# bdwsq1996/Effi-MVS-plus

Measured on NVIDIA B200. Metric: depth_maps_per_sec_1600x1184_5view, higher is better.
Workload: dtype hi+lo bf16 MMA x3, f32 accumulate (3-D regularization, fp32-grade) / f32 (warp, lookup, regression)

## Files before the change

### effi-mvs-plus_b200/capi.py

```python
from __future__ import annotations

import ctypes as C
import os

_HERE = os.path.dirname(os.path.abspath(__file__))
LIB_PATH = os.environ.get("EFFIMVS_LIB") or os.path.join(_HERE, "libeffimvs.so")

OK, EINVAL, EUNSUPPORTED, ECUDA, EWORKSPACE = 0, -1, -2, -3, -4
HYP_TENSOR, HYP_PLANES, HYP_LOCAL = 0, 1, 2
RANGE_SCALAR, RANGE_PIXEL = 0, 1
FEA_NCHW, FEA_NHWC = 0, 1
PREC_F32, PREC_BF16, PREC_BF16X3 = 0, 1, 2
WS_PREPARE, WS_RUN = 1, 2
CONV2D_BIAS, CONV2D_BIAS_RELU, CONV2D_ADD_RELU, CONV2D_GRU_GATES, CONV2D_GRU_UPDATE = 0, 1, 2, 3, 4
MAX_SRC_VIEWS = 16


class EffiMVSError(RuntimeError):
    def __init__(self, code, msg):
        super().__init__("libeffimvs error {}: {}".format(code, msg))
        self.code = code


if not os.path.exists(LIB_PATH):
# ... 34 lines not shown
    "effimvs_inv_init_f32": (_i, [_p, _p, _p, _i, _i, _p, _p, _p]),
    "effimvs_delta_head_f32": (_i, [_p, _p, _p, _p, _p, _p, _i, _i, _i, _i, _p, _p, _p]),
    "effimvs_convex_upsample_f32": (_i, [_p, _p, _f, _p, _p, _p, _i, _i, _i, _i, _p, _p, _p]),
    "effimvs_convex_upsample_conv_f32": (_i, [_p, _i, _p, _p, _f, _p, _p, _p, _i, _i, _i, _i, _p, _p, _p]),
    "effimvs_encoder_head_f32": (_i, [_p, _p, _p, _p, _p, _p, _i, _i, _i, _i, _i, _p, _p]),
    "effimvs_encoder_head_hostw_f32": (_i, [_p, _p, _p, _i, _i, _i, _i, _i, _p, _p]),
    "effimvs_encoder_head_pack_host": (_i, [_p, _p, _p, _p, _i, _i, _p]),
    "effimvs_encoder_head_table_floats": (_i, [_i]),
    "effimvs_encoder_tail_f32": (_i, [_p, _p, _p, C.c_longlong, _i, _i, _p, _p]),
    "effimvs_encoder_tail_ctx_f32": (_i, [_p, _p, _p, _i, _i, _i, _p, _p, C.c_longlong, _i, _i, _p, _p]),
    "effimvs_conv2d_tf32_supported": (_i, [_i, _i]),
    "effimvs_conv2d_tf32_packed_bytes": (_sz, [_i, _i]),
    "effimvs_conv2d_tf32_pack": (_i, [_p, _i, _i, _p, _p]),
    "effimvs_conv2d_tf32": (_i, [_p, C.c_longlong, _i, _p, C.c_longlong, _i, _p, _p, _i, _i, _i, _i, _i,
                                 _p, C.c_longlong, _p, C.c_longlong, _p, C.c_longlong, _p]),
    "effimvs_gru_init_f32": (_i, [_p, C.c_longlong, _i, _i, _p, _p]),
    "effimvs_gru_init_ctx_f32": (_i, [_p, C.c_longlong, _i, _i, _p, _p, _p, _p, _p]),
    "effimvs_dtu_filter_f32": (_i, [_p, _p, _p, _p, C.POINTER(C.c_double), C.POINTER(C.c_float), _i, _i, _i, _f, _f, _i, _i, _i,
                                    _p, _p, _p, _p, _p, _p, _p]),
    "effimvs_images_u8_to_f32": (_i, [_p, C.c_longlong, _p, _p]),
    "effimvs_fusion_invert_cameras_f32": (_i, [_p, _p, _i, _i, _p, _p]),
    "effimvs_fusion_reproject_f32": (_i, [_p, _p, _p, _p, _p, _i, _i, _i, _i, _p, _p]),
    "effimvs_fusion_filter_f32": (_i, [_p, _p, _p, _p, _p, _p, _i, _i, _i, _i, _i, _i, _f, _f, _i, _f, _i, _p, _p, _p, _p, _p]),
}

for _name, (_res, _args) in SIGNATURES.items():
    _fn = getattr(lib, _name)
    _fn.restype = _res
    _fn.argtypes = _args

# ... 14 lines not shown
```

### effi-mvs-plus_b200/csrc/common.cuh

```cuda
#pragma once
#include <cuda_runtime.h>
#include <stdint.h>
#include <stdio.h>

#include <utility>

#include "../../include/effimvs.h"

namespace effimvs {

void set_error(const char* fmt, ...);

inline int check_launch(const char* what) {
    cudaError_t e = cudaGetLastError();
    if (e != cudaSuccess) {
        set_error("%s: %s", what, cudaGetErrorString(e));
        return EFFIMVS_ECUDA;
    }
    return EFFIMVS_OK;
}

#define EFFI_REQUIRE(cond, code, ...)      \
    do {                                   \
        if (!(cond)) {                     \
// ... 30 lines not shown
template <class... KArgs, class... Args>
inline void launch_kernel(void (*kernel)(KArgs...), dim3 grid, dim3 block, size_t smem, cudaStream_t stream, Args&&... args) {
    cudaLaunchConfig_t cfg = {};
    cfg.gridDim = grid;
    cfg.blockDim = block;
    cfg.dynamicSmemBytes = smem;
    cfg.stream = stream;
    cudaLaunchAttribute attr[1];
    attr[0].id = cudaLaunchAttributeProgrammaticStreamSerialization;
    attr[0].val.programmaticStreamSerializationAllowed = 1;
    cfg.attrs = attr;
    cfg.numAttrs = pdl_enabled() ? 1 : 0;
    cudaLaunchKernelEx(&cfg, kernel, std::forward<Args>(args)...);
}

struct SrcPtrs {
    const float* p[EFFIMVS_MAX_SRC_VIEWS];
};

}
```

### effi-mvs-plus_b200/csrc/conv2d_tc.cu

```cuda
#include <cuda_fp16.h>

#include <algorithm>
#include <cstdlib>

#include "common.cuh"

namespace effimvs {
namespace {

constexpr int C2_TM = 128;
constexpr int C2_ROWPX = 136;
constexpr int C2_CG_BYTES = C2_ROWPX * 16;
constexpr int C2_STAGES = 4;
constexpr int C2_RING = 16;
constexpr int C2_PROD_WARPS = 8;
constexpr int C2_PROD_GROUPS = 2;
constexpr int C2_GROUP_WARPS = C2_PROD_WARPS / C2_PROD_GROUPS;
constexpr int C2_MMA_WARP = 4, C2_PROD_WARP0 = 5;
constexpr int C2_THREADS = (C2_PROD_WARP0 + C2_PROD_WARPS) * 32;
constexpr int C2_EPI_STRIDE = 144;
constexpr int C2_EPI_BYTES = 4 * 32 * C2_EPI_STRIDE;
constexpr int C2_MAX_COUT = 128;

struct C2Params {
// ... 2 lines not shown
    int cin, cout, coutp;
    int B, H, W;
    int kc, n_phases;
    int strips, R, chunks, n_units;
    int mode;
    const float* bias;
    float* out; long long out_ps;
    const float* aux0; long long aux0_ps;
    float* aux1; long long aux1_ps;
    int tmem_cols, w_bytes, stage_bytes, n_stages;
    int gw;
    int ring;
    long long* tl;
    int debug;
};

__device__ __forceinline__ uint32_t smem_u32(const void* p) { return (uint32_t)__cvta_generic_to_shared(p); }
__device__ __forceinline__ void mbar_init(uint64_t* bar, uint32_t count) {
    asm volatile("mbarrier.init.shared::cta.b64 [%0], %1;" ::"r"(smem_u32(bar)), "r"(count));
}
__device__ __forceinline__ void mbar_expect_tx(uint64_t* bar, uint32_t bytes) {
    asm volatile("mbarrier.arrive.expect_tx.shared::cta.b64 _, [%0], %1;" ::"r"(smem_u32(bar)), "r"(bytes) : "memory");
}
__device__ __forceinline__ void mbar_arrive(uint64_t* bar) {
    asm volatile("mbarrier.arrive.shared::cta.b64 _, [%0];" ::"r"(smem_u32(bar)) : "memory");
}
__device__ __forceinline__ uint32_t mbar_try(uint64_t* bar, uint32_t parity) {
    uint32_t done;
    asm volatile(
        "{\n\t.reg .pred p;\n\t"
// ... 200 lines not shown
}

struct Unit { int b, y0, y1, x0; };
__device__ __forceinline__ Unit unit_of(const C2Params& P, int u) {
    Unit t;
    const int per_img = P.strips * P.chunks;
    t.b = u / per_img;
    const int r = u - t.b * per_img;
    const int chunk = r / P.strips, strip = r - chunk * P.strips;
    t.y0 = chunk * P.R;
    t.y1 = min(t.y0 + P.R, P.H);
    t.x0 = strip * C2_TM;
    return t;
}

template <int MODE, int GROUPS>
__global__ void __launch_bounds__(C2_THREADS, 2)
conv2d_tc_kernel(const __grid_constant__ C2Params P, const uint8_t* __restrict__ wpk) {
#ifdef EFFIMVS_CONV2D_PROFILING
    const int dbg = dbg;
#else
    constexpr int dbg = 0;
#endif
    constexpr int KC = GROUPS * 8;
    extern __shared__ __align__(128) uint8_t smem[];
    __shared__ __align__(8) uint64_t bar_afull[C2_STAGES], bar_aempty[C2_STAGES], bar_tfull[C2_RING], bar_tempty[C2_RING], bar_w;
    __shared__ uint32_t tmem_base_s;
    __shared__ __align__(16) float sbias[C2_MAX_COUT];
    const int tid = threadIdx.x, warp = __shfl_sync(0xffffffffu, tid >> 5, 0), lane = tid & 31;
    uint8_t* wsm = smem;
    uint8_t* astage = smem + P.w_bytes;

    if (warp == C2_MMA_WARP) {
// ... 4 lines not shown
        for (int s = 0; s < C2_STAGES; ++s) { mbar_init(&bar_afull[s], P.gw); mbar_init(&bar_aempty[s], 1); }
        for (int a = 0; a < C2_RING; ++a) { mbar_init(&bar_tfull[a], 1); mbar_init(&bar_tempty[a], 4); }
        mbar_init(&bar_w, 1);
        asm volatile("fence.mbarrier_init.release.cluster;" ::: "memory");
    }
    tc_fence_before();
    __syncthreads();
    tc_fence_after();
    if (tid == C2_PROD_WARP0 * 32) {
        mbar_expect_tx(&bar_w, (uint32_t)P.w_bytes);
        bulk_g2s(wsm, wpk, (uint32_t)P.w_bytes, &bar_w);
    }
    pdl_trigger();
    pdl_wait();
    if (tid < C2_MAX_COUT) sbias[tid] = (P.bias && tid < P.cout) ? __ldg(P.bias + tid) : 0.0f;
    __syncthreads();
    const uint32_t tmem = tmem_base_s;
    const int H = P.H, W = P.W;

    if (warp >= C2_PROD_WARP0) {
        const int pw = warp - C2_PROD_WARP0, grp = pw / P.gw, pwg = pw - grp * P.gw;
        const int S = P.n_stages;
        constexpr int groups = GROUPS;
        const int pxl = groups >= 4 ? (lane & 7) : (lane & 15), cgl0 = groups >= 4 ? (lane >> 3) : (lane >> 4);
        const int px_per_item = groups >= 4 ? 8 : 16, px_items = (C2_ROWPX + px_per_item - 1) / px_per_item;
        const int n_items = px_items * (groups >= 4 ? groups >> 2 : 1);
        const int ps0i = (int)P.ps0, ps1i = (int)P.ps1;
        uint32_t fill = 0;
        for (int u = blockIdx.x; u < P.n_units; u += gridDim.x) {
            const Unit t = unit_of(P, u);
            const int i_lo = max(t.y0 - 1, 0), i_hi = min(t.y1, H - 1);
            for (int i = i_lo; i <= i_hi; ++i) {
                const long long rowpix = ((long long)t.b * H + i) * W;
                for (int p = 0; p < P.n_phases; ++p, ++fill) {
                    if ((int)(fill % C2_PROD_GROUPS) != grp) continue;
// ... 212 lines not shown
        dst[i] = __float2half_rn(fminf(fmaxf(v, -65504.0f), 65504.0f));
    }
}

int pow2_cols(int n) { int c = 32; while (c < n) c <<= 1; return c; }
int phase_channels(int cin) { return (cin == 16 || cin == 32 || cin == 64) ? cin : (cin % 32 == 0 ? 32 : 16); }

}
}

using namespace effimvs;

static long long* g_conv2d_timeline = nullptr;
extern "C" void effimvs_conv2d_debug_timeline(void* buf) { g_conv2d_timeline = (long long*)buf; }

extern "C" size_t effimvs_conv2d_tf32_packed_bytes(int cin, int cout) {
    if (cin <= 0 || cout <= 0) return 0;
    const int coutp = (cout + 15) / 16 * 16;
    return (size_t)18 * cin * coutp;
}

extern "C" int effimvs_conv2d_tf32_supported(int cin, int cout) {
    if (cin < 16 || cin % 16 != 0 || cout < 4 || cout % 4 != 0 || cout > C2_MAX_COUT) return 0;
    const int coutp = (cout + 15) / 16 * 16;
    const int kc = phase_channels(cin);
    const size_t smem = (size_t)18 * cin * coutp + (size_t)3 * (kc / 8) * C2_CG_BYTES + C2_EPI_BYTES;
    if (smem > 224 * 1024) return 0;
    if (4 * coutp > 512) return 0;
    return 1;
}

extern "C" int effimvs_conv2d_tf32_pack(const float* w, int cin, int cout, void* packed, void* stream) {
    EFFI_REQUIRE(w && packed, EFFIMVS_EINVAL, "conv2d_tf32_pack: null pointer");
    EFFI_REQUIRE(effimvs_conv2d_tf32_supported(cin, cout), EFFIMVS_EUNSUPPORTED, "conv2d_tf32_pack: cin=%d cout=%d not supported", cin, cout);
    const int coutp = (cout + 15) / 16 * 16;
    const int total = 9 * cin * coutp;
    conv2d_pack_kernel<<<std::min(ceil_div(total, 256), 1024), 256, 0, (cudaStream_t)stream>>>(w, cin, cout, coutp, (__half*)packed);
    return check_launch("conv2d_pack_kernel");
}

extern "C" int effimvs_conv2d_tf32(const float* in0, long long in0_ps, int c0, const float* in1, long long in1_ps, int c1,
                                   const void* packed, const float* bias, int cout, int B, int H, int W, int mode,
                                   float* out, long long out_ps, const float* aux0, long long aux0_ps, float* aux1,
                                   long long aux1_ps, void* stream) {
    EFFI_REQUIRE(in0 && packed && out, EFFIMVS_EINVAL, "conv2d_tf32: null pointer");
    EFFI_REQUIRE(B > 0 && H >= 2 && W >= 1, EFFIMVS_EINVAL, "conv2d_tf32: bad shape %dx%dx%d", B, H, W);
    EFFI_REQUIRE(c0 > 0 && c0 % 8 == 0 && c1 >= 0 && c1 % 8 == 0 && (c1 == 0 || in1), EFFIMVS_EINVAL, "conv2d_tf32: bad channel segments %d + %d", c0, c1);
    const int cin = c0 + c1;
    EFFI_REQUIRE(effimvs_conv2d_tf32_supported(cin, cout), EFFIMVS_EUNSUPPORTED, "conv2d_tf32: cin=%d cout=%d not supported", cin, cout);
    EFFI_REQUIRE(mode >= EFFIMVS_CONV2D_BIAS && mode <= EFFIMVS_CONV2D_GRU_UPDATE, EFFIMVS_EINVAL, "conv2d_tf32: bad mode %d", mode);
    EFFI_REQUIRE(in0_ps >= c0 && in0_ps % 8 == 0 && (c1 == 0 || (in1_ps >= c1 && in1_ps % 8 == 0)) && out_ps % 4 == 0,
                 EFFIMVS_EINVAL, "conv2d_tf32: input pixel strides must be multiples of 8 floats, the output's of 4");
    EFFI_REQUIRE((((uintptr_t)in0 | (uintptr_t)in1) & 31) == 0 && (((uintptr_t)out | (uintptr_t)aux0 | (uintptr_t)aux1 | (uintptr_t)packed) & 15) == 0,
                 EFFIMVS_EINVAL, "conv2d_tf32: input maps must be 32-byte aligned, the other pointers 16-byte aligned");
    EFFI_REQUIRE((long long)W * in0_ps < (1ll << 31) && (long long)W * in1_ps < (1ll << 31), EFFIMVS_EUNSUPPORTED, "conv2d_tf32: a row of a map must be below 2^31 floats");
    if (mode == EFFIMVS_CONV2D_ADD_RELU) EFFI_REQUIRE(aux0 && aux0_ps % 4 == 0, EFFIMVS_EINVAL, "conv2d_tf32: ADD_RELU needs the addend map");
    if (mode == EFFIMVS_CONV2D_GRU_GATES)
        EFFI_REQUIRE(aux0 && aux1 && bias && cout % 32 == 0 && aux0_ps % 4 == 0 && aux1_ps % 4 == 0, EFFIMVS_EINVAL,
                     "conv2d_tf32: GRU_GATES needs h_prev, the z buffer, the bias and cout = 2h with h a multiple of 16");
    if (mode == EFFIMVS_CONV2D_GRU_UPDATE) EFFI_REQUIRE(aux0 && bias && aux0_ps % 4 == 0, EFFIMVS_EINVAL, "conv2d_tf32: GRU_UPDATE needs z and the bias");

    C2Params P;
    P.in0 = in0; P.ps0 = in0_ps; P.c0 = c0;
    P.in1 = in1 ? in1 : in0; P.ps1 = in1 ? in1_ps : in0_ps; P.c1 = c1;
    P.cin = cin; P.cout = cout; P.coutp = (cout + 15) / 16 * 16;
    P.B = B; P.H = H; P.W = W;
    P.kc = phase_channels(cin);
    P.n_phases = cin / P.kc;
    P.mode = mode;
    P.tl = g_conv2d_timeline;
    P.debug = getenv("EFFIMVS_CONV2D_DEBUG") ? atoi(getenv("EFFIMVS_CONV2D_DEBUG")) : 0;
    P.bias = bias;
    P.out = out; P.out_ps = out_ps;
    P.aux0 = aux0; P.aux0_ps = aux0_ps;
    P.aux1 = aux1; P.aux1_ps = aux1_ps;
    P.w_bytes = 18 * cin * P.coutp;
    P.stage_bytes = (P.kc / 8) * C2_CG_BYTES;
    const size_t fixed = (size_t)P.w_bytes + C2_EPI_BYTES;
    const size_t smem3 = fixed + 3 * (size_t)P.stage_bytes;
    int per_sm = smem3 + 1024 <= 75 * 1024 && 4 * P.coutp <= 128 ? 3 : (smem3 + 1024 <= 113 * 1024 && 4 * P.coutp <= 256 ? 2 : 1);
    if (const char* e = getenv("EFFIMVS_CONV2D_CTAS")) per_sm = std::max(1, std::min(per_sm, atoi(e)));
    P.gw = per_sm == 3 ? 2 : 4;
    const int tmem_budget = per_sm == 3 ? 128 : (per_sm == 2 ? 256 : 512);
    P.ring = 4;
    while (P.ring < C2_RING && 2 * P.ring * P.coutp <= tmem_budget) P.ring *= 2;
    if (const char* e = getenv("EFFIMVS_CONV2D_RING")) { int r = atoi(e); if ((r == 4 || r == 8 || r == 16) && r * P.coutp <= tmem_budget) P.ring = r; }
    P.tmem_cols = pow2_cols(P.ring * P.coutp);
    const size_t smem_budget = per_sm == 3 ? 75 * 1024 : (per_sm == 2 ? 113 * 1024 : 225 * 1024);
    P.n_stages = (smem3 + P.stage_bytes + 1024 <= smem_budget) ? 4 : 3;
    if (const char* e = getenv("EFFIMVS_CONV2D_STAGES")) { int n = atoi(e); if (n == 3 || (n == 4 && smem3 + P.stage_bytes + 1024 <= smem_budget)) P.n_stages = n; }
    const size_t smem = fixed + (size_t)P.n_stages * P.stage_bytes;
    const int G = kNumSMs * per_sm;
    P.strips = ceil_div(W, C2_TM);
    int chunks = std::max(1, (G + B * P.strips / 2) / (B * P.strips));
    if (const char* e = getenv("EFFIMVS_CONV2D_ROWS")) chunks = ceil_div(H, std::max(1, atoi(e)));
    int min_rows = 4;
    if (const char* e = getenv("EFFIMVS_CONV2D_MINROWS")) min_rows = std::max(1, atoi(e));
    P.R = std::max(std::min(min_rows, H), ceil_div(H, chunks));
    P.chunks = ceil_div(H, P.R);
    P.n_units = B * P.strips * P.chunks;

    typedef void (*KernelFn)(C2Params, const uint8_t*);
#define C2_ROW(M) {conv2d_tc_kernel<M, 2>, conv2d_tc_kernel<M, 4>, conv2d_tc_kernel<M, 8>}
    static const KernelFn table[5][3] = {C2_ROW(EFFIMVS_CONV2D_BIAS), C2_ROW(EFFIMVS_CONV2D_BIAS_RELU), C2_ROW(EFFIMVS_CONV2D_ADD_RELU),
                                         C2_ROW(EFFIMVS_CONV2D_GRU_GATES), C2_ROW(EFFIMVS_CONV2D_GRU_UPDATE)};
#undef C2_ROW
    const int gi = P.kc == 16 ? 0 : (P.kc == 32 ? 1 : 2);
    const KernelFn fn = table[mode][gi];
    static bool attr_set[64][5][3] = {};
    int dev = 0;
    cudaGetDevice(&dev);
    if (dev < 0 || dev >= 64 || !attr_set[dev][mode][gi]) {
        cudaError_t e = cudaFuncSetAttribute(fn, cudaFuncAttributeMaxDynamicSharedMemorySize, 226 * 1024);
        EFFI_REQUIRE(e == cudaSuccess, EFFIMVS_ECUDA, "conv2d_tf32: cudaFuncSetAttribute: %s", cudaGetErrorString(e));
        if (dev >= 0 && dev < 64) attr_set[dev][mode][gi] = true;
    }
    launch_kernel(fn, dim3(std::min(G, P.n_units)), dim3((C2_PROD_WARP0 + C2_PROD_GROUPS * P.gw) * 32), smem, (cudaStream_t)stream, P,
                  (const uint8_t*)packed);
    return check_launch("conv2d_tc_kernel");
}
```

### effi-mvs-plus_b200/csrc/update_glue.cu

```cuda
#include <stdlib.h>

#include "common.cuh"

namespace effimvs {
namespace {

__device__ __forceinline__ float sigmoid_t(float x) { return __fdiv_rn(1.0f, __fadd_rn(1.0f, expf(-x))); }

__device__ __forceinline__ float to_depth(float inv, float lo, float hi) {
    const float s = fmaxf(__fadd_rn(lo, __fmul_rn(__fsub_rn(hi, lo), inv)), 1e-4f);
    return __fdiv_rn(1.0f, s);
}

__global__ void __launch_bounds__(256)
gru_reset_kernel(const float4* __restrict__ zr_pre, const float* __restrict__ bias_r, const float4* __restrict__ hx, long long n_pix, int h,
                 int cx, float4* __restrict__ rhx) {
    pdl_enter();
    const int ct4 = (h + cx) >> 2, h4 = h >> 2;
    const long long total = n_pix * ct4;
    for (long long i = (long long)blockIdx.x * blockDim.x + threadIdx.x; i < total; i += (long long)gridDim.x * blockDim.x) {
        const long long p = i / ct4;
        const int c4 = (int)(i - p * ct4);
        float4 v = __ldg(hx + i);
        if (c4 < h4) {
// ... 412 lines not shown
                        acc[p][4 * q + 2] = fmaf(v[tx + p], wv.z, acc[p][4 * q + 2]); acc[p][4 * q + 3] = fmaf(v[tx + p], wv.w, acc[p][4 * q + 3]);
                    }
                }
            }
        }
#pragma unroll
        for (int p = 0; p < EH_PX; ++p)
            if (has[p])
#pragma unroll
                for (int q = 0; q < 4; ++q)
                    o[p][((h + ch) >> 2) + q] = make_float4(fmaxf(acc[p][4 * q], 0.0f), fmaxf(acc[p][4 * q + 1], 0.0f), fmaxf(acc[p][4 * q + 2], 0.0f),
                                                            fmaxf(acc[p][4 * q + 3], 0.0f));
    }
}

struct EHTable {
    float wd[49][16];
    float wc[8][16];
    float bc[16], bd[16];
};
static_assert(sizeof(EHTable) == 944 * sizeof(float), "EHTable layout is part of the C ABI (effimvs_encoder_head_pack_host)");

template <int EH_TY>
__global__ void __launch_bounds__(EH_TX * EH_TY)
encoder_head_const_kernel(const __grid_constant__ EHTable T, const float* __restrict__ cost, int CD, const float* __restrict__ inv,
                          int h, int ch0, int H, int W, float* __restrict__ out) {
    constexpr int TWP = EH_TX * EH_PX, SW = TWP + 2 * EH_R, SH = EH_TY + 2 * EH_R;
    static_assert(SW % 2 == 0 && EH_PX == 2, "window rows are read as float2 pairs");
    __shared__ __align__(16) float s_inv[SH * SW];
    pdl_enter();
    const int b = blockIdx.z;
    const int x0 = blockIdx.x * TWP - EH_R, y0 = blockIdx.y * EH_TY - EH_R;
    const float* ib = inv + (size_t)b * H * W;
    for (int r = threadIdx.y; r < SH; r += EH_TY) {
        const int yy = y0 + r;
        const bool rok = yy >= 0 && yy < H;
// ... 355 lines not shown
```

### effi-mvs-plus_b200/hotpath.py

```python
from __future__ import annotations

import collections
import os
import weakref

import torch

from . import capi, ops


def fold_bn(block, transposed: bool):
    bn = block.bn
    scale = bn.weight / torch.sqrt(bn.running_var + bn.eps)
    shift = bn.bias - bn.running_mean * scale
    w = block.conv.weight
    w = w * (scale.reshape(1, -1, 1, 1, 1) if transposed else scale.reshape(-1, 1, 1, 1, 1))
    return w.detach().float().contiguous(), shift.detach().float().contiguous()


class _FoldCache:

    def __init__(self):
        self._store = weakref.WeakKeyDictionary()

# ... 206 lines not shown
    gru_update = staticmethod(ops.gru_update)
    gru_delta = staticmethod(ops.gru_delta)
    inv_init = staticmethod(ops.inv_init)
    depth_ranges = staticmethod(ops.depth_ranges)
    delta_head = staticmethod(ops.delta_head)
    convex_upsample = staticmethod(ops.convex_upsample)
    convex_upsample_conv = staticmethod(ops.convex_upsample_conv)
    encoder_head = staticmethod(ops.encoder_head)
    encoder_tail = staticmethod(ops.encoder_tail)
    encoder_tail_ctx = staticmethod(ops.encoder_tail_ctx)
    gru_init = staticmethod(ops.gru_init)
    gru_init_ctx = staticmethod(ops.gru_init_ctx)
    conv2d_tc = staticmethod(ops.conv2d_tc)
    conv2d_tc_pack = staticmethod(ops.conv2d_tc_pack)
    conv2d_tc_supported = staticmethod(ops.conv2d_tc_supported)

    def softmax_regress_conf(self, prob_pre, hyp):
        if _is_planes(hyp):
            B, D = prob_pre.shape[:2]
            return ops.softmax_regress_conf(prob_pre, hyp.reshape(B, D, -1)[:, :, 0].contiguous(), capi.HYP_PLANES)
        return ops.softmax_regress_conf(prob_pre, hyp, capi.HYP_TENSOR)
```

### effi-mvs-plus_b200/net.py

```python
from __future__ import annotations

import os

import torch
import torch.nn as nn
import torch.nn.functional as F

_FUSED_CONV_RELU = os.environ.get("EFFIMVS_FUSED_CONV_RELU", "1") == "1"


def conv_relu(x, weight, bias, stride=(1, 1), padding=(0, 0)):
    if _FUSED_CONV_RELU and x.is_cuda and bias is not None and not torch.is_grad_enabled():
        return torch.cudnn_convolution_relu(x, weight, bias, stride, padding, (1, 1), 1)
    return F.relu(F.conv2d(x, weight, bias, stride, padding), inplace=True)


def _conv_relu_mod(conv: nn.Conv2d, x):
    return conv_relu(x, conv.weight, conv.bias, conv.stride, conv.padding)


class ConvBNReLU2d(nn.Module):

    def __init__(self, cin, cout, k, stride=1, padding=0):
        super().__init__()
# ... 278 lines not shown
        inv_depth = (cur_depth.reciprocal() - lo) / ((hi - lo) + 1e-10)
    return glue.gru_delta(None, None, inv_depth, lo_disp, hi_disp)


def _update_block_forward_tc(block, glue, w, hx, ctx_term, cost_fn, inv_depth, iters, lo_disp, hi_disp, want_mask, cur_depth=None):
    from . import capi
    g, e, hd = block.depth_gru, block.encoder, block.depth_head
    tc = _tc_update_weights(block, glue, w)
    B, two_h, H, W = hx.shape
    h = two_h // 2
    ratio = int(round((block.mask[2].out_channels / 9) ** 0.5))
    mk = lambda c: torch.empty(B, c, H, W, device=hx.device, dtype=torch.float32, memory_format=torch.channels_last)
    cd, z, rh, t1 = mk(two_h), mk(h), mk(h), mk(h)
    net_v, x_v = hx[:, :h], hx[:, h:]
    cd2_cudnn = os.environ.get("EFFIMVS_CONV2D_CD2", "own") == "cudnn"
    inv, depth = _start_inverse_depth(glue, inv_depth, cur_depth, lo_disp, hi_disp)
    inv_seq, depth_seq = [], []
    for it in range(iters):
        c1d1 = glue.encoder_head(cost_fn(depth, it), inv, e.convc1.weight, e.convc1.bias, e.convd1.weight, e.convd1.bias)
        if cd2_cudnn:
            cd = conv_relu(c1d1, w["w_cd2"], w["b_cd2"], (1, 1), (1, 1))
        else:
            glue.conv2d_tc(c1d1, None, tc["cd2"], w["b_cd2"], two_h, capi.CONV2D_BIAS_RELU, cd, None, None)
        glue.conv2d_tc(cd, None, tc["dprime"], None, h, capi.CONV2D_ADD_RELU, x_v, ctx_term, None)
        glue.conv2d_tc(hx, None, tc["zr"], tc["b_zr"], two_h, capi.CONV2D_GRU_GATES, rh, net_v, z)
        glue.conv2d_tc(rh, x_v, tc["q"], g.convq.bias, h, capi.CONV2D_GRU_UPDATE, net_v, z, None)
        glue.conv2d_tc(net_v, None, tc["head1"], hd.conv1.bias, h, capi.CONV2D_BIAS_RELU, t1, None, None)
        inv, depth = glue.delta_head(t1, w["w_d2"], hd.conv2.bias, inv, lo_disp, hi_disp)
        inv_seq.append(inv)
        depth_seq.append(depth)
    m0 = mk(two_h)
    glue.conv2d_tc(net_v, None, tc["mask0"], block.mask[0].bias, two_h, capi.CONV2D_BIAS_RELU, m0, None, None)
    mask_pre = F.conv2d(m0, block.mask[2].weight, None)
    up, depth_up = glue.convex_upsample(mask_pre, block.mask[2].bias, 0.25, inv, lo_disp, hi_disp, ratio)
    return net_v, inv_seq, depth_seq, up, depth_up, (mask_pre if want_mask else None)


def update_block_forward_fused(block, glue, net, cost_fn, inv_depth, context, iters, lo_disp, hi_disp, ctx_map=None, want_mask=True,
# ... 216 lines not shown
```

### effi-mvs-plus_b200/ops.py

```python
from __future__ import annotations

import os
from typing import List, Optional, Tuple

import torch
from torch import Tensor

from . import capi

_lib = capi.lib
_NHWC_MAXC = int(os.environ.get("EFFIMVS_NHWC_MAXC", "32"))

LAUNCHES = 0


def _count(n: int) -> None:
    global LAUNCHES
    LAUNCHES += n


def _dev(t: Tensor, name: str) -> Tensor:
    if not t.is_cuda:
        raise RuntimeError("effimvs::{} got a CPU tensor; the hot path is CUDA-only (no fallback)".format(name))
    if t.dtype != torch.float32:
# ... 856 lines not shown
        if a is not None and tuple(a.shape) != (B, h, H, W):
            raise ValueError("conv2d_tc: aux map {} should be {}".format(tuple(a.shape), (B, h, H, W)))
    if packed.numel() * 4 != _lib.effimvs_conv2d_tf32_packed_bytes(c0 + c1, cout):
        raise ValueError("conv2d_tc: packed weights do not match cin = {} cout = {}".format(c0 + c1, cout))
    bias = _dev(bias, "conv2d_tc") if bias is not None else None
    _count(1)
    capi.check(_lib.effimvs_conv2d_tf32(p0, ps0, c0, p1, ps1, c1, packed.data_ptr(), _opt(bias), cout, B, H, W, mode,
                                        po, pso, pa0, psa0, pa1, psa1, _stream()))


@conv2d_tc.register_fake
def _(in0, in1, packed, bias, cout, mode, out, aux0, aux1):
    return None


@torch.library.custom_op("effimvs::gru_init", mutates_args=())
@_on_tensor_device
def gru_init(ctx_map: Tensor, h: int) -> Tensor:
    ctx_map = _nhwc(ctx_map, "gru_init")
    B, ct, H, W = ctx_map.shape
    if h <= 0 or h % 4 or ct < h or (ct - h) % 4:
        raise ValueError("gru_init: hidden {} / map channels {} must be multiples of 4".format(h, ct))
    hx = torch.empty(B, 2 * h, H, W, device=ctx_map.device, dtype=torch.float32, memory_format=torch.channels_last)
    _count(1)
    capi.check(_lib.effimvs_gru_init_f32(ctx_map.data_ptr(), B * H * W, h, ct - h, hx.data_ptr(), _stream()))
    return hx


@gru_init.register_fake
def _(ctx_map, h):
# ... 66 lines not shown
```

### include/effimvs.h

```cpp
#ifndef EFFIMVS_H
#define EFFIMVS_H

#include <stddef.h>
#include <stdint.h>

#ifdef __cplusplus
extern "C" {
#endif

#define EFFIMVS_OK 0
#define EFFIMVS_EINVAL (-1)
#define EFFIMVS_EUNSUPPORTED (-2)
#define EFFIMVS_ECUDA (-3)
#define EFFIMVS_EWORKSPACE (-4)

#define EFFIMVS_MAX_SRC_VIEWS 16

#define EFFIMVS_HYP_TENSOR 0
#define EFFIMVS_HYP_PLANES 1
#define EFFIMVS_HYP_LOCAL 2

#define EFFIMVS_FEA_NCHW 0
#define EFFIMVS_FEA_NHWC 1

// ... 134 lines not shown
                             float* hx, float* ctx_term, void* stream);

#define EFFIMVS_CONV2D_BIAS 0
#define EFFIMVS_CONV2D_BIAS_RELU 1
#define EFFIMVS_CONV2D_ADD_RELU 2
#define EFFIMVS_CONV2D_GRU_GATES 3
#define EFFIMVS_CONV2D_GRU_UPDATE 4

int effimvs_conv2d_tf32_supported(int cin, int cout);
size_t effimvs_conv2d_tf32_packed_bytes(int cin, int cout);
int effimvs_conv2d_tf32_pack(const float* w, int cin, int cout, void* packed, void* stream);
int effimvs_conv2d_tf32(const float* in0, long long in0_pixstride, int c0, const float* in1, long long in1_pixstride, int c1,
                        const void* packed, const float* bias, int cout, int B, int H, int W, int mode,
                        float* out, long long out_pixstride, const float* aux0, long long aux0_pixstride,
                        float* aux1, long long aux1_pixstride, void* stream);

int effimvs_dtu_filter_f32(const float* ref_depth, const float* srcs_depth, const float* conf, const float* mats,
                           const double* thr_dist_host, const float* thr_diff_host, int n_rungs, int first_rung,
                           int full_count, float conf_thres, float conf_keep, int v, int h, int w,
                           uint8_t* final_mask, uint8_t* geo_mask, float* depth_avg, float* points, uint8_t* masks_out,
                           float* reproj_depth_out, void* stream);

#ifdef __cplusplus
}
#endif
#endif
```

Baseline: 165.6.

## Fuse encoder head convolutions into the cd2 tensor-core conv producer warps

The encoder head (1x1 cost conv and 7x7 inverse-depth conv with ReLU) is now computed inside the producer warps of the tensor-core conv2d kernel, written straight into the shared-memory A stages as half precision, instead of being materialised in global memory by a separate kernel. This removes one kernel launch per GRU iteration and the write and re-read of the c1d1 intermediate map. In exchange the producer warps do much more FMA work per row and the kernel needs extra shared memory for weight tables and input tiles, which may lower CTAs per SM or starve the MMA consumer.

Measured after the change: 147.8 (median of 6 runs). -10.8%, worse.

```diff
diff --git a/effi-mvs-plus_b200/capi.py b/effi-mvs-plus_b200/capi.py
--- a/effi-mvs-plus_b200/capi.py
+++ b/effi-mvs-plus_b200/capi.py
@@ -72,6 +72,7 @@
     "effimvs_conv2d_tf32_pack": (_i, [_p, _i, _i, _p, _p]),
     "effimvs_conv2d_tf32": (_i, [_p, C.c_longlong, _i, _p, C.c_longlong, _i, _p, _p, _i, _i, _i, _i, _i,
                                  _p, C.c_longlong, _p, C.c_longlong, _p, C.c_longlong, _p]),
+    "effimvs_encoder_conv2d_tf32": (_i, [_p, _p, _p, _p, _p, _p, _i, _i, _i, _i, _i, _p, _p, _p, C.c_longlong, _p]),
     "effimvs_gru_init_f32": (_i, [_p, C.c_longlong, _i, _i, _p, _p]),
     "effimvs_gru_init_ctx_f32": (_i, [_p, C.c_longlong, _i, _i, _p, _p, _p, _p, _p]),
     "effimvs_dtu_filter_f32": (_i, [_p, _p, _p, _p, C.POINTER(C.c_double), C.POINTER(C.c_float), _i, _i, _i, _f, _f, _i, _i, _i,
diff --git a/effi-mvs-plus_b200/csrc/common.cuh b/effi-mvs-plus_b200/csrc/common.cuh
--- a/effi-mvs-plus_b200/csrc/common.cuh
+++ b/effi-mvs-plus_b200/csrc/common.cuh
@@ -68,6 +68,13 @@
     cudaLaunchKernelEx(&cfg, kernel, std::forward<Args>(args)...);
 }
 
+struct EHTable {
+    float wd[49][16];
+    float wc[8][16];
+    float bc[16], bd[16];
+};
+static_assert(sizeof(EHTable) == 944 * sizeof(float), "EHTable layout is part of the C ABI (effimvs_encoder_head_pack_host)");
+
 struct SrcPtrs {
     const float* p[EFFIMVS_MAX_SRC_VIEWS];
 };
diff --git a/effi-mvs-plus_b200/csrc/conv2d_tc.cu b/effi-mvs-plus_b200/csrc/conv2d_tc.cu
--- a/effi-mvs-plus_b200/csrc/conv2d_tc.cu
+++ b/effi-mvs-plus_b200/csrc/conv2d_tc.cu
@@ -40,6 +40,18 @@
     long long* tl;
     int debug;
 };
+
+struct NoHead { static constexpr int NCH = 0; };
+template <int NCH_>
+struct EHProducer {
+    static constexpr int NCH = NCH_;
+    const float *cost, *inv;
+    const float *wc1, *bc1, *wd1, *bd1;
+    int CD;
+};
+constexpr int EH_TW = 40;
+constexpr int EH_TILE_BYTES = 7 * EH_TW * 4;
+constexpr int EH_TILES_BYTES = C2_PROD_WARPS * EH_TILE_BYTES;
 
 __device__ __forceinline__ uint32_t smem_u32(const void* p) { return (uint32_t)__cvta_generic_to_shared(p); }
 __device__ __forceinline__ void mbar_init(uint64_t* bar, uint32_t count) {
@@ -270,9 +282,108 @@
     return t;
 }
 
-template <int MODE, int GROUPS>
+__device__ __forceinline__ uint32_t pack_half2f(float lo, float hi) {
+    uint32_t r;
+    asm("cvt.rn.satfinite.f16x2.f32 %0, %1, %2;" : "=r"(r) : "f"(hi), "f"(lo));
+    return r;
+}
+__device__ __forceinline__ void eh_store16(uint8_t* d, const float (&a)[16], bool inside) {
+    uint32_t q[8];
+#pragma unroll
+    for (int e = 0; e < 8; ++e) q[e] = inside ? pack_half2f(fmaxf(a[2 * e], 0.0f), fmaxf(a[2 * e + 1], 0.0f)) : 0u;
+    *reinterpret_cast<uint4*>(d) = make_uint4(q[0], q[1], q[2], q[3]);
+    *reinterpret_cast<uint4*>(d + C2_CG_BYTES) = make_uint4(q[4], q[5], q[6], q[7]);
+}
+
+template <int NCH>
+__device__ __forceinline__ void eh_fill(const C2Params& P, const EHProducer<NCH>& E, const EHTable* __restrict__ st, uint8_t* dst,
+                                        float* tile, const Unit& t, int i, int pwg, int lane) {
+    constexpr int h = 16 * NCH;
+    const int H = P.H, W = P.W, CD = E.CD;
+    const long long plane = (long long)H * W;
+    const float* inv_b = E.inv + (long long)t.b * plane;
+    const float* cost_r = E.cost + (long long)t.b * CD * plane + (long long)i * W;
+    for (int blk = pwg; blk < 4; blk += P.gw) {
+        const int xb = t.x0 - 1 + blk * 32, x = xb + lane;
+        uint8_t* d = dst + (blk * 32 + lane) * 16;
+        if (xb >= W) {
+#pragma unroll
+            for (int cg = 0; cg < h / 4; ++cg) *reinterpret_cast<uint4*>(d + cg * C2_CG_BYTES) = make_uint4(0u, 0u, 0u, 0u);
+            continue;
+        }
+        const bool inside = x >= 0 && x < W;
+        float cv[8];
+#pragma unroll
+        for (int c = 0; c < 8; ++c) cv[c] = (c < CD && inside) ? __ldg(cost_r + c * plane + x) : 0.0f;
+#pragma unroll
+        for (int r = 0; r < 7; ++r) {
+            const int yy = i - 3 + r, xa = xb - 3 + lane, xc = xa + 32;
+            const bool rok = (unsigned)yy < (unsigned)H;
+            const float* rowp = inv_b + (long long)(rok ? yy : 0) * W;
+            tile[r * EH_TW + lane] = (rok && (unsigned)xa < (unsigned)W) ? __ldg(rowp + xa) : 0.0f;
+            if (lane < 6) tile[r * EH_TW + 32 + lane] = (rok && (unsigned)xc < (unsigned)W) ? __ldg(rowp + xc) : 0.0f;
+        }
+        __syncwarp();
+#pragma unroll
+        for (int k = 0; k < NCH; ++k) {
+            const EHTable& T = st[k];
+            float a[16];
+#pragma unroll
+            for (int j = 0; j < 16; ++j) a[j] = T.bc[j];
+#pragma unroll
+            for (int c = 0; c < 8; ++c)
+                if (c < CD)
+#pragma unroll
+                    for (int j = 0; j < 16; ++j) a[j] = fmaf(cv[c], T.wc[c][j], a[j]);
+            eh_store16(d + 2 * k * C2_CG_BYTES, a, inside);
+#pragma unroll
+            for (int j = 0; j < 16; ++j) a[j] = T.bd[j];
+#pragma unroll
+            for (int ty = 0; ty < 7; ++ty) {
+                float v[7];
+#pragma unroll
+                for (int tx = 0; tx < 7; ++tx) v[tx] = tile[ty * EH_TW + lane + tx];
+#pragma unroll
+                for (int tx = 0; tx < 7; ++tx)
+#pragma unroll
+                    for (int j = 0; j < 16; ++j) a[j] = fmaf(v[tx], T.wd[ty * 7 + tx][j], a[j]);
+            }
+            eh_store16(d + (h / 8 + 2 * k) * C2_CG_BYTES, a, inside);
+        }
+        __syncwarp();
+    }
+    for (int task = pwg * 32 + lane; task < 4 * h; task += P.gw * 32) {
+        const int oc = task >> 1, px = C2_TM + (task & 1), x = t.x0 - 1 + px;
+        float a = 0.0f;
+        if (x < W) {
+            if (oc < h) {
+                a = __ldg(E.bc1 + oc);
+                for (int c = 0; c < CD; ++c) a = fmaf(__ldg(cost_r + c * plane + x), __ldg(E.wc1 + oc * CD + c), a);
+            } else {
+                const float* wd = E.wd1 + (oc - h) * 49;
+                a = __ldg(E.bd1 + oc - h);
+#pragma unroll
+                for (int ty = 0; ty < 7; ++ty) {
+                    const int yy = i - 3 + ty;
+                    const bool rok = (unsigned)yy < (unsigned)H;
+                    const float* rowp = inv_b + (long long)(rok ? yy : 0) * W;
+#pragma unroll
+                    for (int tx = 0; tx < 7; ++tx) {
+                        const int xx = x - 3 + tx;
+                        const float v = (rok && (unsigned)xx < (unsigned)W) ? __ldg(rowp + xx) : 0.0f;
+                        a = fmaf(v, __ldg(wd + ty * 7 + tx), a);
+                    }
+                }
+            }
+            a = fmaxf(a, 0.0f);
+        }
+        *reinterpret_cast<uint16_t*>(dst + (oc >> 3) * C2_CG_BYTES + px * 16 + (oc & 7) * 2) = (uint16_t)(pack_half2f(a, 0.0f) & 0xffffu);
+    }
+}
+
+template <int MODE, int GROUPS, class HEAD>
 __global__ void __launch_bounds__(C2_THREADS, 2)
-conv2d_tc_kernel(const __grid_constant__ C2Params P, const uint8_t* __restrict__ wpk) {
+conv2d_tc_kernel(const __grid_constant__ C2Params P, const uint8_t* __restrict__ wpk, const __grid_constant__ HEAD E) {
 #ifdef EFFIMVS_CONV2D_PROFILING
     const int dbg = dbg;
 #else
@@ -307,11 +418,45 @@
     pdl_trigger();
     pdl_wait();
     if (tid < C2_MAX_COUT) sbias[tid] = (P.bias && tid < P.cout) ? __ldg(P.bias + tid) : 0.0f;
+    EHTable* stab = reinterpret_cast<EHTable*>(astage + (size_t)P.n_stages * P.stage_bytes + C2_EPI_BYTES + EH_TILES_BYTES);
+    if constexpr (HEAD::NCH > 0) {
+        float* sw = reinterpret_cast<float*>(stab);
+        for (int idx = tid; idx < HEAD::NCH * 944; idx += blockDim.x) {
+            const int k = idx / 944, r = idx - k * 944, j = r & 15, ch = k * 16 + j;
+            float v;
+            if (r < 784) v = __ldg(E.wd1 + ch * 49 + (r >> 4));
+            else if (r < 912) v = ((r - 784) >> 4) < E.CD ? __ldg(E.wc1 + ch * E.CD + ((r - 784) >> 4)) : 0.0f;
+            else if (r < 928) v = __ldg(E.bc1 + ch);
+            else v = __ldg(E.bd1 + ch);
+            sw[idx] = v;
+        }
+    }
     __syncthreads();
     const uint32_t tmem = tmem_base_s;
     const int H = P.H, W = P.W;
 
-    if (warp >= C2_PROD_WARP0) {
+    if (HEAD::NCH > 0 && warp >= C2_PROD_WARP0) {
+        if constexpr (HEAD::NCH > 0) {
+            const int pw = warp - C2_PROD_WARP0, grp = pw / P.gw, pwg = pw - grp * P.gw;
+            const int S = P.n_stages;
+            float* tile = reinterpret_cast<float*>(astage + (size_t)S * P.stage_bytes + C2_EPI_BYTES + (size_t)pw * EH_TILE_BYTES);
+            uint32_t fill = 0;
+            for (int u = blockIdx.x; u < P.n_units; u += gridDim.x) {
+                const Unit t = unit_of(P, u);
+                const int i_lo = max(t.y0 - 1, 0), i_hi = min(t.y1, H - 1);
+                for (int i = i_lo; i <= i_hi; ++i, ++fill) {
+                    if ((int)(fill % C2_PROD_GROUPS) != grp) continue;
+                    const uint32_t s = fill % S, n = fill / S;
+                    if (lane == 0) mbar_wait(&bar_aempty[s], (n & 1) ^ 1);
+                    __syncwarp();
+                    eh_fill<HEAD::NCH>(P, E, stab, astage + (size_t)s * P.stage_bytes, tile, t, i, pwg, lane);
+                    fence_async_smem();
+                    __syncwarp();
+                    if (lane == 0) mbar_arrive(&bar_afull[s]);
+                }
+            }
+        }
+    } else if (warp >= C2_PROD_WARP0) {
         const int pw = warp - C2_PROD_WARP0, grp = pw / P.gw, pwg = pw - grp * P.gw;
         const int S = P.n_stages;
         constexpr int groups = GROUPS;
@@ -554,69 +699,15 @@
 static long long* g_conv2d_timeline = nullptr;
 extern "C" void effimvs_conv2d_debug_timeline(void* buf) { g_conv2d_timeline = (long long*)buf; }
 
-extern "C" size_t effimvs_conv2d_tf32_packed_bytes(int cin, int cout) {
-    if (cin <= 0 || cout <= 0) return 0;
-    const int coutp = (cout + 15) / 16 * 16;
-    return (size_t)18 * cin * coutp;
-}
-
-extern "C" int effimvs_conv2d_tf32_supported(int cin, int cout) {
-    if (cin < 16 || cin % 16 != 0 || cout < 4 || cout % 4 != 0 || cout > C2_MAX_COUT) return 0;
-    const int coutp = (cout + 15) / 16 * 16;
-    const int kc = phase_channels(cin);
-    const size_t smem = (size_t)18 * cin * coutp + (size_t)3 * (kc / 8) * C2_CG_BYTES + C2_EPI_BYTES;
-    if (smem > 224 * 1024) return 0;
-    if (4 * coutp > 512) return 0;
-    return 1;
-}
-
-extern "C" int effimvs_conv2d_tf32_pack(const float* w, int cin, int cout, void* packed, void* stream) {
-    EFFI_REQUIRE(w && packed, EFFIMVS_EINVAL, "conv2d_tf32_pack: null pointer");
-    EFFI_REQUIRE(effimvs_conv2d_tf32_supported(cin, cout), EFFIMVS_EUNSUPPORTED, "conv2d_tf32_pack: cin=%d cout=%d not supported", cin, cout);
-    const int coutp = (cout + 15) / 16 * 16;
-    const int total = 9 * cin * coutp;
-    conv2d_pack_kernel<<<std::min(ceil_div(total, 256), 1024), 256, 0, (cudaStream_t)stream>>>(w, cin, cout, coutp, (__half*)packed);
-    return check_launch("conv2d_pack_kernel");
-}
-
-extern "C" int effimvs_conv2d_tf32(const float* in0, long long in0_ps, int c0, const float* in1, long long in1_ps, int c1,
-                                   const void* packed, const float* bias, int cout, int B, int H, int W, int mode,
-                                   float* out, long long out_ps, const float* aux0, long long aux0_ps, float* aux1,
-                                   long long aux1_ps, void* stream) {
-    EFFI_REQUIRE(in0 && packed && out, EFFIMVS_EINVAL, "conv2d_tf32: null pointer");
-    EFFI_REQUIRE(B > 0 && H >= 2 && W >= 1, EFFIMVS_EINVAL, "conv2d_tf32: bad shape %dx%dx%d", B, H, W);
-    EFFI_REQUIRE(c0 > 0 && c0 % 8 == 0 && c1 >= 0 && c1 % 8 == 0 && (c1 == 0 || in1), EFFIMVS_EINVAL, "conv2d_tf32: bad channel segments %d + %d", c0, c1);
-    const int cin = c0 + c1;
-    EFFI_REQUIRE(effimvs_conv2d_tf32_supported(cin, cout), EFFIMVS_EUNSUPPORTED, "conv2d_tf32: cin=%d cout=%d not supported", cin, cout);
-    EFFI_REQUIRE(mode >= EFFIMVS_CONV2D_BIAS && mode <= EFFIMVS_CONV2D_GRU_UPDATE, EFFIMVS_EINVAL, "conv2d_tf32: bad mode %d", mode);
-    EFFI_REQUIRE(in0_ps >= c0 && in0_ps % 8 == 0 && (c1 == 0 || (in1_ps >= c1 && in1_ps % 8 == 0)) && out_ps % 4 == 0,
-                 EFFIMVS_EINVAL, "conv2d_tf32: input pixel strides must be multiples of 8 floats, the output's of 4");
-    EFFI_REQUIRE((((uintptr_t)in0 | (uintptr_t)in1) & 31) == 0 && (((uintptr_t)out | (uintptr_t)aux0 | (uintptr_t)aux1 | (uintptr_t)packed) & 15) == 0,
-                 EFFIMVS_EINVAL, "conv2d_tf32: input maps must be 32-byte aligned, the other pointers 16-byte aligned");
-    EFFI_REQUIRE((long long)W * in0_ps < (1ll << 31) && (long long)W * in1_ps < (1ll << 31), EFFIMVS_EUNSUPPORTED, "conv2d_tf32: a row of a map must be below 2^31 floats");
-    if (mode == EFFIMVS_CONV2D_ADD_RELU) EFFI_REQUIRE(aux0 && aux0_ps % 4 == 0, EFFIMVS_EINVAL, "conv2d_tf32: ADD_RELU needs the addend map");
-    if (mode == EFFIMVS_CONV2D_GRU_GATES)
-        EFFI_REQUIRE(aux0 && aux1 && bias && cout % 32 == 0 && aux0_ps % 4 == 0 && aux1_ps % 4 == 0, EFFIMVS_EINVAL,
-                     "conv2d_tf32: GRU_GATES needs h_prev, the z buffer, the bias and cout = 2h with h a multiple of 16");
-    if (mode == EFFIMVS_CONV2D_GRU_UPDATE) EFFI_REQUIRE(aux0 && bias && aux0_ps % 4 == 0, EFFIMVS_EINVAL, "conv2d_tf32: GRU_UPDATE needs z and the bias");
-
-    C2Params P;
-    P.in0 = in0; P.ps0 = in0_ps; P.c0 = c0;
-    P.in1 = in1 ? in1 : in0; P.ps1 = in1 ? in1_ps : in0_ps; P.c1 = c1;
-    P.cin = cin; P.cout = cout; P.coutp = (cout + 15) / 16 * 16;
-    P.B = B; P.H = H; P.W = W;
-    P.kc = phase_channels(cin);
-    P.n_phases = cin / P.kc;
-    P.mode = mode;
+static size_t c2_configure(C2Params& P, size_t extra_smem, int& grid) {
+    const int B = P.B, H = P.H, W = P.W;
     P.tl = g_conv2d_timeline;
     P.debug = getenv("EFFIMVS_CONV2D_DEBUG") ? atoi(getenv("EFFIMVS_CONV2D_DEBUG")) : 0;
-    P.bias = bias;
-    P.out = out; P.out_ps = out_ps;
-    P.aux0 = aux0; P.aux0_ps = aux0_ps;
-    P.aux1 = aux1; P.aux1_ps = aux1_ps;
-    P.w_bytes = 18 * cin * P.coutp;
+    P.kc = phase_channels(P.cin);
+    P.n_phases = P.cin / P.kc;
+    P.w_bytes = 18 * P.cin * P.coutp;
     P.stage_bytes = (P.kc / 8) * C2_CG_BYTES;
-    const size_t fixed = (size_t)P.w_bytes + C2_EPI_BYTES;
+    const size_t fixed = (size_t)P.w_bytes + C2_EPI_BYTES + extra_smem;
     const size_t smem3 = fixed + 3 * (size_t)P.stage_bytes;
     int per_sm = smem3 + 1024 <= 75 * 1024 && 4 * P.coutp <= 128 ? 3 : (smem3 + 1024 <= 113 * 1024 && 4 * P.coutp <= 256 ? 2 : 1);
     if (const char* e = getenv("EFFIMVS_CONV2D_CTAS")) per_sm = std::max(1, std::min(per_sm, atoi(e)));
@@ -639,23 +730,128 @@
     P.R = std::max(std::min(min_rows, H), ceil_div(H, chunks));
     P.chunks = ceil_div(H, P.R);
     P.n_units = B * P.strips * P.chunks;
-
-    typedef void (*KernelFn)(C2Params, const uint8_t*);
-#define C2_ROW(M) {conv2d_tc_kernel<M, 2>, conv2d_tc_kernel<M, 4>, conv2d_tc_kernel<M, 8>}
+    grid = std::min(G, P.n_units);
+    return smem;
+}
+
+template <class K>
+static int c2_allow_smem(K fn, bool (&done)[64]) {
+    int dev = 0;
+    cudaGetDevice(&dev);
+    if (dev >= 0 && dev < 64 && done[dev]) return EFFIMVS_OK;
+    cudaError_t e = cudaFuncSetAttribute(fn, cudaFuncAttributeMaxDynamicSharedMemorySize, 226 * 1024);
+    EFFI_REQUIRE(e == cudaSuccess, EFFIMVS_ECUDA, "conv2d_tf32: cudaFuncSetAttribute: %s", cudaGetErrorString(e));
+    if (dev >= 0 && dev < 64) done[dev] = true;
+    return EFFIMVS_OK;
+}
+
+extern "C" size_t effimvs_conv2d_tf32_packed_bytes(int cin, int cout) {
+    if (cin <= 0 || cout <= 0) return 0;
+    const int coutp = (cout + 15) / 16 * 16;
+    return (size_t)18 * cin * coutp;
+}
+
+extern "C" int effimvs_conv2d_tf32_supported(int cin, int cout) {
+    if (cin < 16 || cin % 16 != 0 || cout < 4 || cout % 4 != 0 || cout > C2_MAX_COUT) return 0;
+    const int coutp = (cout + 15) / 16 * 16;
+    const int kc = phase_channels(cin);
+    const size_t smem = (size_t)18 * cin * coutp + (size_t)3 * (kc / 8) * C2_CG_BYTES + C2_EPI_BYTES;
+    if (smem > 224 * 1024) return 0;
+    if (4 * coutp > 512) return 0;
+    return 1;
+}
+
+extern "C" int effimvs_conv2d_tf32_pack(const float* w, int cin, int cout, void* packed, void* stream) {
+    EFFI_REQUIRE(w && packed, EFFIMVS_EINVAL, "conv2d_tf32_pack: null pointer");
+    EFFI_REQUIRE(effimvs_conv2d_tf32_supported(cin, cout), EFFIMVS_EUNSUPPORTED, "conv2d_tf32_pack: cin=%d cout=%d not supported", cin, cout);
+    const int coutp = (cout + 15) / 16 * 16;
+    const int total = 9 * cin * coutp;
+    conv2d_pack_kernel<<<std::min(ceil_div(total, 256), 1024), 256, 0, (cudaStream_t)stream>>>(w, cin, cout, coutp, (__half*)packed);
+    return check_launch("conv2d_pack_kernel");
+}
+
+extern "C" int effimvs_conv2d_tf32(const float* in0, long long in0_ps, int c0, const float* in1, long long in1_ps, int c1,
+                                   const void* packed, const float* bias, int cout, int B, int H, int W, int mode,
+                                   float* out, long long out_ps, const float* aux0, long long aux0_ps, float* aux1,
+                                   long long aux1_ps, void* stream) {
+    EFFI_REQUIRE(in0 && packed && out, EFFIMVS_EINVAL, "conv2d_tf32: null pointer");
+    EFFI_REQUIRE(B > 0 && H >= 2 && W >= 1, EFFIMVS_EINVAL, "conv2d_tf32: bad shape %dx%dx%d", B, H, W);
+    EFFI_REQUIRE(c0 > 0 && c0 % 8 == 0 && c1 >= 0 && c1 % 8 == 0 && (c1 == 0 || in1), EFFIMVS_EINVAL, "conv2d_tf32: bad channel segments %d + %d", c0, c1);
+    const int cin = c0 + c1;
+    EFFI_REQUIRE(effimvs_conv2d_tf32_supported(cin, cout), EFFIMVS_EUNSUPPORTED, "conv2d_tf32: cin=%d cout=%d not supported", cin, cout);
+    EFFI_REQUIRE(mode >= EFFIMVS_CONV2D_BIAS && mode <= EFFIMVS_CONV2D_GRU_UPDATE, EFFIMVS_EINVAL, "conv2d_tf32: bad mode %d", mode);
+    EFFI_REQUIRE(in0_ps >= c0 && in0_ps % 8 == 0 && (c1 == 0 || (in1_ps >= c1 && in1_ps % 8 == 0)) && out_ps % 4 == 0,
+                 EFFIMVS_EINVAL, "conv2d_tf32: input pixel strides must be multiples of 8 floats, the output's of 4");
+    EFFI_REQUIRE((((uintptr_t)in0 | (uintptr_t)in1) & 31) == 0 && (((uintptr_t)out | (uintptr_t)aux0 | (uintptr_t)aux1 | (uintptr_t)packed) & 15) == 0,
+                 EFFIMVS_EINVAL, "conv2d_tf32: input maps must be 32-byte aligned, the other pointers 16-byte aligned");
+    EFFI_REQUIRE((long long)W * in0_ps < (1ll << 31) && (long long)W * in1_ps < (1ll << 31), EFFIMVS_EUNSUPPORTED, "conv2d_tf32: a row of a map must be below 2^31 floats");
+    if (mode == EFFIMVS_CONV2D_ADD_RELU) EFFI_REQUIRE(aux0 && aux0_ps % 4 == 0, EFFIMVS_EINVAL, "conv2d_tf32: ADD_RELU needs the addend map");
+    if (mode == EFFIMVS_CONV2D_GRU_GATES)
+        EFFI_REQUIRE(aux0 && aux1 && bias && cout % 32 == 0 && aux0_ps % 4 == 0 && aux1_ps % 4 == 0, EFFIMVS_EINVAL,
+                     "conv2d_tf32: GRU_GATES needs h_prev, the z buffer, the bias and cout = 2h with h a multiple of 16");
+    if (mode == EFFIMVS_CONV2D_GRU_UPDATE) EFFI_REQUIRE(aux0 && bias && aux0_ps % 4 == 0, EFFIMVS_EINVAL, "conv2d_tf32: GRU_UPDATE needs z and the bias");
+
+    C2Params P;
+    P.in0 = in0; P.ps0 = in0_ps; P.c0 = c0;
+    P.in1 = in1 ? in1 : in0; P.ps1 = in1 ? in1_ps : in0_ps; P.c1 = c1;
+    P.cin = cin; P.cout = cout; P.coutp = (cout + 15) / 16 * 16;
+    P.B = B; P.H = H; P.W = W;
+    P.mode = mode;
+    P.bias = bias;
+    P.out = out; P.out_ps = out_ps;
+    P.aux0 = aux0; P.aux0_ps = aux0_ps;
+    P.aux1 = aux1; P.aux1_ps = aux1_ps;
+    int grid = 0;
+    const size_t smem = c2_configure(P, 0, grid);
+    typedef void (*KernelFn)(C2Params, const uint8_t*, NoHead);
+#define C2_ROW(M) {conv2d_tc_kernel<M, 2, NoHead>, conv2d_tc_kernel<M, 4, NoHead>, conv2d_tc_kernel<M, 8, NoHead>}
     static const KernelFn table[5][3] = {C2_ROW(EFFIMVS_CONV2D_BIAS), C2_ROW(EFFIMVS_CONV2D_BIAS_RELU), C2_ROW(EFFIMVS_CONV2D_ADD_RELU),
                                          C2_ROW(EFFIMVS_CONV2D_GRU_GATES), C2_ROW(EFFIMVS_CONV2D_GRU_UPDATE)};
 #undef C2_ROW
     const int gi = P.kc == 16 ? 0 : (P.kc == 32 ? 1 : 2);
     const KernelFn fn = table[mode][gi];
-    static bool attr_set[64][5][3] = {};
-    int dev = 0;
-    cudaGetDevice(&dev);
-    if (dev < 0 || dev >= 64 || !attr_set[dev][mode][gi]) {
-        cudaError_t e = cudaFuncSetAttribute(fn, cudaFuncAttributeMaxDynamicSharedMemorySize, 226 * 1024);
-        EFFI_REQUIRE(e == cudaSuccess, EFFIMVS_ECUDA, "conv2d_tf32: cudaFuncSetAttribute: %s", cudaGetErrorString(e));
-        if (dev >= 0 && dev < 64) attr_set[dev][mode][gi] = true;
-    }
-    launch_kernel(fn, dim3(std::min(G, P.n_units)), dim3((C2_PROD_WARP0 + C2_PROD_GROUPS * P.gw) * 32), smem, (cudaStream_t)stream, P,
-                  (const uint8_t*)packed);
+    static bool attr_set[5][3][64] = {};
+    if (int rc = c2_allow_smem(fn, attr_set[mode][gi])) return rc;
+    launch_kernel(fn, dim3(grid), dim3((C2_PROD_WARP0 + C2_PROD_GROUPS * P.gw) * 32), smem, (cudaStream_t)stream, P,
+                  (const uint8_t*)packed, NoHead{});
     return check_launch("conv2d_tc_kernel");
 }
+
+template <int NCH>
+static int encoder_conv2d_launch(const C2Params& P0, const float* cost, const float* inv, const float* wc1,
+                                 const float* bc1, const float* wd1, const float* bd1, int CD, const void* packed, cudaStream_t stream) {
+    C2Params P = P0;
+    int grid = 0;
+    const size_t smem = c2_configure(P, EH_TILES_BYTES + NCH * sizeof(EHTable), grid);
+    EHProducer<NCH> E;
+    E.cost = cost; E.inv = inv;
+    E.wc1 = wc1; E.bc1 = bc1; E.wd1 = wd1; E.bd1 = bd1;
+    E.CD = CD;
+    const auto fn = conv2d_tc_kernel<EFFIMVS_CONV2D_BIAS_RELU, NCH * 4, EHProducer<NCH>>;
+    static bool attr_set[64] = {};
+    if (int rc = c2_allow_smem(fn, attr_set)) return rc;
+    launch_kernel(fn, dim3(grid), dim3((C2_PROD_WARP0 + C2_PROD_GROUPS * P.gw) * 32), smem, stream, P, (const uint8_t*)packed, E);
+    return check_launch("conv2d_tc_kernel<encoder head>");
+}
+
+extern "C" int effimvs_encoder_conv2d_tf32(const float* cost, const float* inv, const float* wc1,
+                                           const float* bc1, const float* wd1, const float* bd1, int B, int CD, int h, int H, int W,
+                                           const void* packed, const float* bias, float* out, long long out_ps, void* stream) {
+    EFFI_REQUIRE(cost && inv && wc1 && bc1 && wd1 && bd1 && packed && out, EFFIMVS_EINVAL, "encoder_conv2d_tf32: null pointer");
+    EFFI_REQUIRE(CD >= 1 && CD <= 8 && (h == 16 || h == 32), EFFIMVS_EUNSUPPORTED,
+                 "encoder_conv2d_tf32: cost channels %d must be in [1,8], hidden %d 16 or 32", CD, h);
+    EFFI_REQUIRE(B > 0 && H >= 2 && W >= 1, EFFIMVS_EINVAL, "encoder_conv2d_tf32: bad shape %dx%dx%d", B, H, W);
+    EFFI_REQUIRE(out_ps >= 2 * h && out_ps % 4 == 0, EFFIMVS_EINVAL, "encoder_conv2d_tf32: output pixel stride %lld must be >= 2h and a multiple of 4", out_ps);
+    EFFI_REQUIRE((((uintptr_t)out | (uintptr_t)packed) & 15) == 0 && (((uintptr_t)cost | (uintptr_t)inv) & 3) == 0, EFFIMVS_EINVAL,
+                 "encoder_conv2d_tf32: output and packed weights must be 16-byte aligned, cost and inv 4-byte aligned");
+    C2Params P = {};
+    P.in0 = P.in1 = cost;
+    P.c0 = 2 * h; P.c1 = 0;
+    P.cin = 2 * h; P.cout = 2 * h; P.coutp = 2 * h;
+    P.B = B; P.H = H; P.W = W;
+    P.mode = EFFIMVS_CONV2D_BIAS_RELU;
+    P.bias = bias;
+    P.out = out; P.out_ps = out_ps;
+    if (h == 16) return encoder_conv2d_launch<1>(P, cost, inv, wc1, bc1, wd1, bd1, CD, packed, (cudaStream_t)stream);
+    return encoder_conv2d_launch<2>(P, cost, inv, wc1, bc1, wd1, bd1, CD, packed, (cudaStream_t)stream);
+}
diff --git a/effi-mvs-plus_b200/csrc/update_glue.cu b/effi-mvs-plus_b200/csrc/update_glue.cu
--- a/effi-mvs-plus_b200/csrc/update_glue.cu
+++ b/effi-mvs-plus_b200/csrc/update_glue.cu
@@ -450,12 +450,6 @@
     }
 }
 
-struct EHTable {
-    float wd[49][16];
-    float wc[8][16];
-    float bc[16], bd[16];
-};
-static_assert(sizeof(EHTable) == 944 * sizeof(float), "EHTable layout is part of the C ABI (effimvs_encoder_head_pack_host)");
 
 template <int EH_TY>
 __global__ void __launch_bounds__(EH_TX * EH_TY)
diff --git a/effi-mvs-plus_b200/hotpath.py b/effi-mvs-plus_b200/hotpath.py
--- a/effi-mvs-plus_b200/hotpath.py
+++ b/effi-mvs-plus_b200/hotpath.py
@@ -244,6 +244,7 @@
     conv2d_tc = staticmethod(ops.conv2d_tc)
     conv2d_tc_pack = staticmethod(ops.conv2d_tc_pack)
     conv2d_tc_supported = staticmethod(ops.conv2d_tc_supported)
+    encoder_conv2d_tc = staticmethod(ops.encoder_conv2d_tc)
 
     def softmax_regress_conf(self, prob_pre, hyp):
         if _is_planes(hyp):
diff --git a/effi-mvs-plus_b200/net.py b/effi-mvs-plus_b200/net.py
--- a/effi-mvs-plus_b200/net.py
+++ b/effi-mvs-plus_b200/net.py
@@ -316,14 +316,19 @@
     cd, z, rh, t1 = mk(two_h), mk(h), mk(h), mk(h)
     net_v, x_v = hx[:, :h], hx[:, h:]
     cd2_cudnn = os.environ.get("EFFIMVS_CONV2D_CD2", "own") == "cudnn"
+    head_in_cd2 = not cd2_cudnn and h in (16, 32) and hasattr(glue, "encoder_conv2d_tc")
     inv, depth = _start_inverse_depth(glue, inv_depth, cur_depth, lo_disp, hi_disp)
     inv_seq, depth_seq = [], []
     for it in range(iters):
-        c1d1 = glue.encoder_head(cost_fn(depth, it), inv, e.convc1.weight, e.convc1.bias, e.convd1.weight, e.convd1.bias)
-        if cd2_cudnn:
-            cd = conv_relu(c1d1, w["w_cd2"], w["b_cd2"], (1, 1), (1, 1))
+        if head_in_cd2:
+            glue.encoder_conv2d_tc(cost_fn(depth, it), inv, e.convc1.weight, e.convc1.bias, e.convd1.weight, e.convd1.bias, tc["cd2"],
+                                   w["b_cd2"], cd)
         else:
-            glue.conv2d_tc(c1d1, None, tc["cd2"], w["b_cd2"], two_h, capi.CONV2D_BIAS_RELU, cd, None, None)
+            c1d1 = glue.encoder_head(cost_fn(depth, it), inv, e.convc1.weight, e.convc1.bias, e.convd1.weight, e.convd1.bias)
+            if cd2_cudnn:
+                cd = conv_relu(c1d1, w["w_cd2"], w["b_cd2"], (1, 1), (1, 1))
+            else:
+                glue.conv2d_tc(c1d1, None, tc["cd2"], w["b_cd2"], two_h, capi.CONV2D_BIAS_RELU, cd, None, None)
         glue.conv2d_tc(cd, None, tc["dprime"], None, h, capi.CONV2D_ADD_RELU, x_v, ctx_term, None)
         glue.conv2d_tc(hx, None, tc["zr"], tc["b_zr"], two_h, capi.CONV2D_GRU_GATES, rh, net_v, z)
         glue.conv2d_tc(rh, x_v, tc["q"], g.convq.bias, h, capi.CONV2D_GRU_UPDATE, net_v, z, None)
diff --git a/effi-mvs-plus_b200/ops.py b/effi-mvs-plus_b200/ops.py
--- a/effi-mvs-plus_b200/ops.py
+++ b/effi-mvs-plus_b200/ops.py
@@ -894,6 +894,32 @@
     return None
 
 
+@torch.library.custom_op("effimvs::encoder_conv2d_tc", mutates_args=("out",))
+@_on_tensor_device
+def encoder_conv2d_tc(cost: Tensor, inv: Tensor, wc1: Tensor, bc1: Tensor, wd1: Tensor, bd1: Tensor, packed: Tensor,
+                      bias: Optional[Tensor], out: Tensor) -> None:
+    cost, inv = _dev(cost, "encoder_conv2d_tc"), _dev(inv, "encoder_conv2d_tc")
+    wc1, bc1, wd1, bd1 = (_dev(t, "encoder_conv2d_tc") for t in (wc1, bc1, wd1, bd1))
+    B, CD, H, W = cost.shape
+    h = wc1.shape[0]
+    if inv.numel() != B * H * W or tuple(out.shape) != (B, 2 * h, H, W):
+        raise ValueError("encoder_conv2d_tc: inv {} / out {} do not match cost {} and h = {}".format(tuple(inv.shape), tuple(out.shape),
+                                                                                                   tuple(cost.shape), h))
+    if packed.numel() * 4 != _lib.effimvs_conv2d_tf32_packed_bytes(2 * h, 2 * h):
+        raise ValueError("encoder_conv2d_tc: packed weights do not match cin = cout = {}".format(2 * h))
+    po, pso = _cl_view(out, "out")
+    bias = _dev(bias, "encoder_conv2d_tc") if bias is not None else None
+    _count(1)
+    capi.check(_lib.effimvs_encoder_conv2d_tf32(cost.data_ptr(), inv.data_ptr(), wc1.data_ptr(), bc1.data_ptr(),
+                                                wd1.data_ptr(), bd1.data_ptr(), B, CD, h, H, W, packed.data_ptr(), _opt(bias),
+                                                po, pso, _stream()))
+
+
+@encoder_conv2d_tc.register_fake
+def _(cost, inv, wc1, bc1, wd1, bd1, packed, bias, out):
+    return None
+
+
 @torch.library.custom_op("effimvs::gru_init", mutates_args=())
 @_on_tensor_device
 def gru_init(ctx_map: Tensor, h: int) -> Tensor:
diff --git a/include/effimvs.h b/include/effimvs.h
--- a/include/effimvs.h
+++ b/include/effimvs.h
@@ -172,6 +172,9 @@
                         const void* packed, const float* bias, int cout, int B, int H, int W, int mode,
                         float* out, long long out_pixstride, const float* aux0, long long aux0_pixstride,
                         float* aux1, long long aux1_pixstride, void* stream);
+int effimvs_encoder_conv2d_tf32(const float* cost, const float* inv, const float* wc1, const float* bc1,
+                                const float* wd1, const float* bd1, int B, int CD, int h, int H, int W, const void* packed,
+                                const float* bias, float* out, long long out_pixstride, void* stream);
 
 int effimvs_dtu_filter_f32(const float* ref_depth, const float* srcs_depth, const float* conf, const float* mats,
                            const double* thr_dist_host, const float* thr_diff_host, int n_rungs, int first_rung,
```
